# Saltfish-AB/LatentSync

Hardware: AMD Instinct MI355X
Metric: lip-synced frames/sec at 256x256, 16-frame window, 20 DDIM steps (higher is better)
Workload: dtype bf16; 1 GPU; configs[1]: 256x256 x16-frame windows, 20 DDIM steps, guidance 1.0, LatentSync-1.5 UNet + SD-VAE, bf16; 48 independent windows of a clip batched per UNet call; windows_per_rank=240, windows_per_batch=48, frames_per_window=16, global_batch=768, resolution=256, parallelism=dp1 (window sharding, RCCL all-gather of decoded frames)

## Files before the change

### latentsync_amd/build.py

```python
import concurrent.futures as cf
import os
import re
import shutil
import subprocess
import sys
import tempfile
import warnings

HERE = os.path.dirname(os.path.abspath(__file__))
REPO = os.path.dirname(HERE)
CSRC = os.path.join(HERE, "csrc")
OBJ = os.path.join(REPO, "build", "obj")
LIB = os.path.join(HERE, "libls_hip.so")
HIPCC = os.environ.get("HIPCC", "/opt/rocm/bin/hipcc")
FLAGS = ["--offload-arch=gfx950", "-O3", "-fPIC", "-std=c++17", "-Wno-unused-result", "-munsafe-fp-atomics",
         "-fno-slp-vectorize"]


def _deps():
    hdrs = [os.path.join(CSRC, f) for f in os.listdir(CSRC) if f.endswith(".h")]
    hdrs.append(os.path.join(REPO, "include", "ls_hip.h"))
    return max(os.path.getmtime(h) for h in hdrs)


COUNTED_VMCNT = ("gemm_rowblock_kernel", "conv_gemm_dma_kernel", "attn5_kernel", "attn8_kernel", "tattn_fused_kernel",
                 "attnw_kernel", "conv3x3_halo_kernel", "ff_chain_kernel")


def _spills(stderr):
    bad, cur = [], None
    for line in stderr.splitlines():
        m = re.search(r"remark: +Function Name: (\S+)", line)
        if m:
            cur = m.group(1)
            continue
        m = re.search(r"remark: +VGPRs Spill: (\d+)", line)
        if m and cur and int(m.group(1)) > 0 and any(k in cur for k in COUNTED_VMCNT):
            bad.append(f"{cur}: {line.split('remark:')[1].strip()}")
    return bad


OBJDUMP = os.environ.get("LLVM_OBJDUMP", "/opt/rocm/lib/llvm/bin/llvm-objdump")
_PK_OPSEL = re.compile(r"v_pk_\w+_f32\b[^\n]*\bop_sel:\[([01,]+)\]")


def _packed_opsel(obj):
    skip = os.environ.get("LS_SKIP_OPSEL_GUARD", "") not in ("", "0")
    if not os.path.exists(OBJDUMP):
        if skip:
            warnings.warn(f"packed-fp32 op_sel guard skipped (LS_SKIP_OPSEL_GUARD): {OBJDUMP} not found")
            return []
        raise RuntimeError(f"packed-fp32 op_sel guard: {OBJDUMP} not found (LS_SKIP_OPSEL_GUARD=1 to build without it)")
    with tempfile.TemporaryDirectory() as td:
        cp = os.path.join(td, "k.o")
        shutil.copy(obj, cp)
        r = subprocess.run([OBJDUMP, "--offloading", cp], capture_output=True, text=True, cwd=td)
        dev = [f for f in os.listdir(td) if "gfx950" in f]
        if r.returncode != 0 or not dev:
            msg = f"could not extract the gfx950 code object of {obj} ({r.stderr.strip()[:200]})"
            if skip:
                warnings.warn("packed-fp32 op_sel guard skipped (LS_SKIP_OPSEL_GUARD): " + msg)
                return []
            raise RuntimeError("packed-fp32 op_sel guard: " + msg + " (LS_SKIP_OPSEL_GUARD=1 to build without it)")
        r = subprocess.run([OBJDUMP, "-d", "--mcpu=gfx950", os.path.join(td, dev[0])], capture_output=True, text=True)
    return [m.group(0).split("//")[0].strip() for m in _PK_OPSEL.finditer(r.stdout) if "1" in m.group(1)]


def _compile(src, obj, dep_time):
    if os.path.exists(obj) and os.path.getmtime(obj) >= max(os.path.getmtime(src), dep_time):
        return obj, None
    cmd = [HIPCC] + FLAGS + ["-Rpass-analysis=kernel-resource-usage", "-c", src, "-o", obj]
    r = subprocess.run(cmd, capture_output=True, text=True)
    if r.returncode != 0:
        return obj, r.stderr
    with open(obj[:-2] + ".remarks", "w") as f:
        f.write(r.stderr)
    bad = _spills(r.stderr)
    if bad:
        os.remove(obj)
        return obj, "register spills in counted-vmcnt kernels:\n" + "\n".join(bad)
    try:
        bad = _packed_opsel(obj)
    except RuntimeError as e:
        os.remove(obj)
        return obj, str(e)
    if bad:
        os.remove(obj)
        return obj, f"{len(bad)} packed-fp32 op_sel instructions (wrong beside MFMAs on gfx950), e.g.:\n" + "\n".join(bad[:4])
    return obj, None


def build(verbose=True):
    os.makedirs(OBJ, exist_ok=True)
    srcs = sorted(os.path.join(CSRC, f) for f in os.listdir(CSRC) if f.endswith(".hip"))
    dep_time = _deps()
    objs = []
    with cf.ThreadPoolExecutor(max_workers=min(8, len(srcs))) as ex:
        futs = [ex.submit(_compile, s, os.path.join(OBJ, os.path.basename(s)[:-4] + ".o"), dep_time) for s in srcs]
        for f in futs:
            obj, err = f.result()
            if err:
                raise RuntimeError(f"hipcc failed for {obj}:\n{err}")
            objs.append(obj)
    if not os.path.exists(LIB) or os.path.getmtime(LIB) < max(os.path.getmtime(o) for o in objs):
        cmd = [HIPCC, "--offload-arch=gfx950", "-shared", "-fPIC", "-o", LIB] + objs
        r = subprocess.run(cmd, capture_output=True, text=True)
        if r.returncode != 0:
            raise RuntimeError("link failed:\n" + r.stderr)
        if verbose:
            print("built", LIB)
    return LIB


if __name__ == "__main__":
    build()
    sys.exit(0)
```

### latentsync_amd/csrc/ls_gemm.hip

```cpp
#include <type_traits>

#include "ls_common.h"

namespace ls {

struct ConvArgs {
  const u16* x1; const u16* x2;
  int C1, C2, Cin, ld1, ld2;
  int n_img, H, W, Ho, Wo, stride, pad, upsample;
  const float* aff_scale; const float* aff_shift; int pix_per_sample; int silu_in;
  const u16* w; int K, N, M, CC;
  const float* bias; const float* rowvec; int rows_per_vec, rowvec_ld, rowvec_mod;
  const float* ln_mr; const float* ln_cs;
  const u16* res; int ldr; float out_scale; int act;
  void* y; int ldy; int y_f32;
  int ktiles, kt_per_split, split; float* partial;
  int ntm, ntn;
  float* stats_out; float stats_eps;
  float* cs_out;
  int ablate;
  int ccm;
  int gm;
  int Mo;
  int phase;
// ... 1642 lines not shown
      if (b == 0 && ci > 0) load_par(ci);
    }
  };
  auto put_halo = [&](int buf, int j0, int j1, const uint4* v_in) __attribute__((always_inline)) {
    uint4* const hb0 = hbuf + buf * HALO;
    float4 gsc[2], gsh[2];
    if constexpr (GN) {
      const float4* gq = gpar + buf * 32 + hc8 * 2;
      gsc[0] = gq[0]; gsc[1] = gq[1]; gsh[0] = gq[16]; gsh[1] = gq[17];
    }
#pragma unroll
    for (int j = j0; j < j1; ++j) {
      if (j * NT + tid >= NPC) continue;
      uint4 v = v_in[j - j0];
      if constexpr (GN) {
        if (hpix[j] >= 0) {
          float f[8];
          unpack8(v, f);
          const float scl[8] = {gsc[0].x, gsc[0].y, gsc[0].z, gsc[0].w, gsc[1].x, gsc[1].y, gsc[1].z, gsc[1].w};
          const float shf[8] = {gsh[0].x, gsh[0].y, gsh[0].z, gsh[0].w, gsh[1].x, gsh[1].y, gsh[1].z, gsh[1].w};
#pragma unroll
          for (int e = 0; e < 8; ++e) f[e] = silu_log2(fmaf(f[e], scl[e], shf[e]));
          v = pack8(f);
        }
      }
      hb0[hdst[j]] = v;
    }
  };
  auto store_halo = [&](int buf, int b) { put_halo(buf, hb_lo(b, NHL), hb_lo(b + 1, NHL), hreg); };

  int wvo[DPT];
#pragma unroll
  for (int j = 0; j < DPT; ++j) {
    const int q = j * NT + tid, row = q >> 3, pc = q & 7;
    const int lc = pc ^ ((row >> 1) & 7);
    wvo[j] = ((q < WSLOT ? row : 0) * a.K + lc * 8) * 2;
  }
  auto wslot = [&](int par, int t) { return PH ? (NSW == 3 ? (par + t) % 3 : t & 1) : NSW == 3 ? t % 3 : (t & 1) ^ par; };
  const int wid_u = __builtin_amdgcn_readfirstlane(wid);
  __builtin_assume(wid_u >= 0 && wid_u < NT / 64);
  lds_u4* const wbuf_l = (lds_u4*)lds_dyn + 2 * HALO;
  lds_u4* const dummy_l = wbuf_l + NSW * WSLOT;
  auto issue_w = [&](int g, int sl) {
    lds_u4* slot = wbuf_l + sl * WSLOT + wid_u * 64;
#pragma unroll
    for (int j = 0; j < DPT; ++j) {
      const bool live = WSLOT % NT == 0 || j * NT + wid_u * 64 < WSLOT;
      ls_raw_buffer_load_lds(rs_w, (__attribute__((address_space(3))) void*)(live ? slot + j * NT : dummy_l), 16, wvo[j],
                             g * 128, 0, 0);
    }
  };

  static_assert(TW == 16, "fragment i = one patch row");
  const int p0 = 64 * wm + l16;
  const int hp0 = (p0 / TW) * P + (p0 % TW) + (COMPACT ? 0 : 3) + py * P + px;

  f32x4 acc[FM][FN];
#pragma unroll
  for (int i = 0; i < FM; ++i)
#pragma unroll
    for (int j = 0; j < FN; ++j) acc[i][j] = (f32x4){0.f, 0.f, 0.f, 0.f};

  for (int g = 0; g < NSW - 1 && g < G; ++g) issue_w(g, g % NSW);
  {
    uint4 hpre[NHL];
    if constexpr (GN) load_par(0);
#pragma unroll
    for (int j = 0; j < NHL; ++j) {
      const int vo = hpix[j] >= 0 ? hpix[j] * a.ld1 * 2 + hc8 * 16 : (int)0x80000000;
      hpre[j] = __builtin_bit_cast(uint4, ls_raw_buffer_load_v4(rs1, vo, 0, 0));
    }
    if constexpr (GN) {
      store_par(0);
      __syncthreads();
    }
    put_halo(0, 0, NHL, hpre);
  }

  bf16x8 apf[2][FM];
  auto read_a = [&](const uint4* hb, int tt) {
    constexpr int TPR = PH ? 2 : 3;
    const int hpt = hp0 + (tt / TPR) * P + tt % TPR;
    const int sw = COMPACT ? (l16 + px + tt % TPR) & 7 : hpt & 7;
#pragma unroll
    for (int ks = 0; ks < 2; ++ks) {
      const int base = hpt * 8 + ((ks * 4 + lg) ^ sw);
#pragma unroll
      for (int i = 0; i < FM; ++i)
        apf[ks][i] = __builtin_bit_cast(bf16x8, hb[base + 8 * (((16 * i) / TW) * P + (16 * i) % TW)]);
    }
  };
  auto tap = [&](int ci, int par, auto t_tag, auto last_tag) {
    constexpr int t = decltype(t_tag)::value;
    constexpr bool LAST = decltype(last_tag)::value;
    const int g = NTAP * ci + t;
    const int hpar = ci & 1;
    constexpr int HY = LAST ? 0 : (t - 1 >= 0 ? halo_issue(t - 1, NHL, GN, TS) : 0) +
                                  (NSW >= 3 && t - 2 >= 0 ? halo_issue(t - 2, NHL, GN, TS) : 0);
    if (g + NSW - 2 >= G) wait_vm<0>();
    else wait_vm<(NSW - 2) * DPT + HY>();
    asm volatile("s_waitcnt lgkmcnt(0)" ::: "memory");
    __builtin_amdgcn_s_barrier();
    asm volatile("" ::: "memory");
    if (g + NSW - 1 < G) issue_w(g + NSW - 1, wslot(par, t + NSW - 1));
    if constexpr (!LAST) {
      if constexpr (GN && t == 1) store_par(ci + 1);
      if constexpr (t == TS || t == 2 * TS) store_halo(hpar ^ 1, t / TS - 1);
      if constexpr (t == 0 || t == TS || t == 2 * TS) load_halo(ci + 1, t / TS);
    }
    const uint4* hb = hbuf + hpar * HALO;
    const uint4* wb = wbuf + wslot(par, t) * WSLOT;
    if constexpr (t == 0) read_a(hb, 0);
#pragma unroll
    for (int ks = 0; ks < 2; ++ks) {
      bf16x8 bfr[FN];
#pragma unroll
      for (int j = 0; j < FN; ++j)
        bfr[j] = __builtin_bit_cast(bf16x8, wb[swz64(wn * WTN + j * 16 + l16, ks * 4 + lg)]);
#pragma unroll
      for (int i = 0; i < FM; ++i)
#pragma unroll
        for (int j = 0; j < FN; ++j)
          acc[i][j] = __builtin_amdgcn_mfma_f32_16x16x32_bf16(apf[ks][i], bfr[j], acc[i][j], 0, 0, 0);
    }
    if constexpr (t < NTAP - 1) read_a(hb, t + 1);
    if constexpr (!LAST && t == NTAP - 1) store_halo(hpar ^ 1, 2);
  };
  using I0 = std::integral_constant<int, 0>; using I1 = std::integral_constant<int, 1>;
  using I2 = std::integral_constant<int, 2>; using I3 = std::integral_constant<int, 3>;
  using I4 = std::integral_constant<int, 4>; using I5 = std::integral_constant<int, 5>;
  using I6 = std::integral_constant<int, 6>; using I7 = std::integral_constant<int, 7>;
  using I8 = std::integral_constant<int, 8>;
  auto chunk = [&](int ci, auto last) {
    const int par = PH && NSW == 3 ? ci % 3 : ci & 1;
    tap(ci, par, I0{}, last); tap(ci, par, I1{}, last); tap(ci, par, I2{}, last);
    tap(ci, par, I3{}, last);
    if constexpr (!PH) {
      tap(ci, par, I4{}, last); tap(ci, par, I5{}, last);
      tap(ci, par, I6{}, last); tap(ci, par, I7{}, last); tap(ci, par, I8{}, last);
    }
  };
  for (int ci = 0; ci + 1 < nchunk; ++ci) chunk(ci, std::false_type{});
  chunk(nchunk - 1, std::true_type{});
  asm volatile("s_waitcnt lgkmcnt(0)" ::: "memory");
  __builtin_amdgcn_s_barrier();
  asm volatile("" ::: "memory");
  const int m0v = PH ? (int)(img * 4 * HW) + ((ph * tpc + tyb) * tpr + txb) * (TH * TW)
                     : (int)(img * HW) + (tyb * tpr + txb) * (TH * TW);
  const long m0r = PH ? img * 4 * HW + (long)(2 * y0 + py) * a.Wo + 2 * x0 + px : img * HW + (long)y0 * a.W + x0;
  static_assert((size_t)(NT / (BN / 8)) * BN * 2 * 4 <= (size_t)2 * HALO * 16, "column-sum partials fit the halo images");
  store_tile_plain<TH * TW, BN, TH / 4, WNW, false, CSF, PH ? -TW : TW, 2>(a, acc, (float*)lds_dyn, m0v, n0, m0r);
}

static bool g_force_regstage = false;
static int g_force_tile = 0, g_force_split = 0;
static int g_ablate = 0;

struct ConvPlan {
  ConvArgs a;
  ls_conv_plan_info i;
  float* cs_pass;
  float* row_stats;
};

template <int V>
using IC = std::integral_constant<int, V>;

template <void (*KERN)(ConvArgs)>
static void launch_plan(const ConvPlan& p, hipStream_t s) {
  if (p.i.lds_bytes) LS_SET_MAX_DYN_SHM(KERN, p.i.lds_bytes);
  KERN<<<p.i.grid, p.i.threads, p.i.lds_bytes, s>>>(p.a);
}

static bool vec_ok(const ConvArgs& a) { return a.N % 8 == 0 && a.ldy % 8 == 0 && (!a.res || a.ldr % 8 == 0); }

struct TileCfg { int bm, bn, split; };

static TileCfg pick_tile(long M, int N, int ktiles, bool allow_split, bool big_ok, int ksize) {
  struct Cand { int bm, bn; double eff; int waves, resident; };
  const Cand cands[] = {{128, 128, 1.0, 4, 2}, {128, 160, 1.2, 4, 2}, {128, 64, 0.72, 4, 2}, {64, 64, 0.42, 4, 4},
                        {128, 32, 0.36, 4, 4}, {256, 256, 1.5, 8, 1}};
  TileCfg best{128, 128, 1};
  double best_t = 1e300;
  for (const Cand& c : cands) {
    if (c.bn == 32 && N > 32) continue;
    if (N <= 32 && c.bn != 32) continue;
    if (c.bm == 256) {
      if (!big_ok || N < 256) continue;
      if (ksize == 1 && ((N % 256 != 0 && N < 1920) || (N < 1280 && N % 160 == 0))) continue;
    }
    if (c.bn == 160 && N % 160 != 0) continue;
    const long tiles = (long)cdiv(M, c.bm) * cdiv(N, c.bn);
    for (int split = 1; split <= 16; ++split) {
      if (split > 1 && (!allow_split || ktiles / split < 4 || tiles >= 256)) break;
      const long blocks = tiles * split;
      const long per_cu = (blocks + 255) / 256;
      const long conc = std::min<long>(c.resident, per_cu);
      const double f = (c.waves * conc >= 8) ? 1.0 : 0.75;
      const double per_block = (double)c.bm * c.bn * 64.0 * cdiv(ktiles, split) / c.eff;
      double t = per_cu * per_block / f;
      if (split > 1) t += (double)M * N * split * 1.5;
      if (t < best_t * 0.97) { best_t = t; best = {c.bm, c.bn, split}; }
    }
  }
  return best;
}

static void set_split(ConvArgs& a, int split) {
  a.kt_per_split = cdiv(a.ktiles, std::max(1, std::min(split, a.ktiles)));
  a.split = cdiv(a.ktiles, a.kt_per_split);
}

static bool g_rowblock = true;
static bool g_rowblock640 = true;
static bool g_rb640_res = false;
static bool g_rb640_fm2 = true;

static bool rowblock_ok(const ls_conv_desc* d, const ConvArgs& a) {
  if (!g_rowblock || g_force_tile || g_force_regstage || d->ksize != 1 || a.C2) return false;
  if (a.aff_scale && (a.ln_mr || a.silu_in || a.pix_per_sample % (a.Cin == 320 ? 256 : 128) ||
                      ((uintptr_t)a.aff_scale | (uintptr_t)a.aff_shift) & 15))
    return false;
  if (!((a.Cin == 320 && a.K == 320 && a.M % 256 == 0) ||
        (g_rowblock640 && a.Cin == 640 && a.K == 640 && a.M % 128 == 0 && (!a.res || g_rb640_res))))
    return false;
  if (a.N % 64 || a.split != 1 || a.y_f32) return false;
  if (a.act != LS_ACT_NONE && a.act != LS_ACT_GEGLU) return false;
  if (a.ldy % 4 || (a.res && a.ldr % 8) || (a.rowvec && (a.rowvec_ld % 4 || a.rows_per_vec % 256))) return false;
  if (((uintptr_t)a.y & 7) || ((uintptr_t)a.res & 15)) return false;
  return (((uintptr_t)a.x1 | (uintptr_t)a.bias | (uintptr_t)a.ln_cs | (uintptr_t)a.rowvec) & 15) == 0;
}

using RowblockInstances =
    std::integer_sequence<int, 0, RB_LN, RB_LN | RB_RV, RB_RES, RB_LN | RB_RES, RB_LN | RB_GEGLU, RB_GEGLU, RB_STATS,
                          RB_RES | RB_STATS, RB_RES | RB_GNCS, RB_AFF, RB_AFF | RB_STATS>;
constexpr int RB_FM1 = RB_STATS | RB_GNCS | RB_AFF;

constexpr size_t rowblock_lds(int kt, int fm, int flags) {
  return (size_t)3 * (16 * 2 * (kt / 2) * 8 + 48 + ((flags & RB_RES) ? 128 * fm * 16 * 2 / 8 : 0)) * 16 +
         ((flags & RB_GNCS) ? 4096 : 0);
}

template <int... F>
static bool rowblock_compiled(int flags, std::integer_sequence<int, F...>) {
  return ((flags == F) || ...);
}

static bool plan_rowblock(ConvPlan& p) {
  ConvArgs& a = p.a;
  const int flags = (a.ln_mr ? RB_LN : 0) | (a.res ? RB_RES : 0) | (a.rowvec ? RB_RV : 0) |
                    (a.act == LS_ACT_GEGLU ? RB_GEGLU : 0) | (a.stats_out ? RB_STATS : 0) | (a.cs_out ? RB_GNCS : 0) |
                    (a.aff_scale ? RB_AFF : 0);
  const int fm = a.K == 320 || (g_rb640_fm2 && !(flags & RB_FM1)) ? 2 : 1, bm = 128 * fm;
  if (a.M % bm || !rowblock_compiled(flags, RowblockInstances{})) return false;
  const int ntm = a.M / bm, nch = a.N / 32;
  const int ntn = std::max(1, std::min(nch, (256 + ntm - 1) / ntm));
  if ((a.stats_out || a.cs_out) && ntn != 1) return false;
  a.ntm = ntm;
  a.ntn = ntn;
  p.i.family = 1;
  p.i.rb_kt = a.K / 32;
  p.i.rb_fm = fm;
  p.i.rb_flags = flags;
  p.i.grid = ntm * ntn;
  p.i.threads = 512;
  p.i.lds_bytes = (int)rowblock_lds(p.i.rb_kt, fm, flags);
  return true;
}

template <int FLAGS>
static void launch_rowblock1(const ConvPlan& p, hipStream_t s) {
  if (p.i.rb_kt == 10) return launch_plan<gemm_rowblock_kernel<10, 2, 2, FLAGS>>(p, s);
  if constexpr (!(FLAGS & RB_FM1)) {
    if (p.i.rb_fm == 2) return launch_plan<gemm_rowblock_kernel<20, 2, 2, FLAGS>>(p, s);
  }
  launch_plan<gemm_rowblock_kernel<20, 1, 2, FLAGS>>(p, s);
}

template <int... F>
static void launch_rowblock(const ConvPlan& p, hipStream_t s, std::integer_sequence<int, F...>) {
  ((p.i.rb_flags == F ? launch_rowblock1<F>(p, s) : void()), ...);
}

constexpr size_t tiled_lds(int bm, int bn, int wm) {
  return std::max<size_t>((size_t)2 * (bm + bn) * 8 * 16, (size_t)(bm / wm) * (bn + 4) * 4);
}

static int epi_kind(const ConvArgs& a) {
  if (a.phase) return EPI_PLAINP;
  if (a.split != 1 || !vec_ok(a) || a.y_f32) return EPI_ANY;
  if (a.act == LS_ACT_NONE) return EPI_PLAIN;
  if (a.act == LS_ACT_GEGLU) return EPI_GEGLU;
  return EPI_ANY;
}

static bool buf_dma_ok(const ConvArgs& a, int ks) {
  if (a.aff_scale) return false;
  if (ks == 1) return a.Cin % 64 == 0 && a.C1 % 64 == 0 && a.K == a.Cin;
  if (a.upsample) return a.Cin % 64 == 0 && a.C1 % 64 == 0 && a.stride == 1 && a.pad == 1;
  return a.Cin % 64 == 0 && a.C1 % 64 == 0 && (a.stride == 1 || a.stride == 2) && (a.pad == 0 || a.pad == 1);
}

template <class B, class F>
static void with_epi(int epi, B buf, F f) {
  switch (epi) {
    case EPI_PLAIN: return f(IC<EPI_PLAIN>{}, buf);
    case EPI_GEGLU: return f(IC<EPI_GEGLU>{}, buf);
    default: return f(IC<EPI_ANY>{}, buf);
  }
}

template <int KS, bool TAPU, class F>
static void with_epi_buf(const ls_conv_plan_info& i, F f) {
  if constexpr (KS == 3 && TAPU) {
    if (i.epi == EPI_PLAINP) return f(IC<EPI_PLAINP>{}, std::true_type{});
  }
  if constexpr (KS == 1 || TAPU) {
    if (i.buf) return with_epi(i.epi, std::true_type{}, f);
  }
  with_epi(i.epi, std::false_type{}, f);
}

template <int BM, int BN, int WM, int WN, int KS, bool TAPU>
static void launch_tiled2(const ConvPlan& p, hipStream_t s) {
  if constexpr (BM != 256) {
    if (p.i.family == 2) return launch_plan<conv_gemm_kernel<BM, BN, WM, WN, KS, TAPU>>(p, s);
  }
  with_epi_buf<KS, TAPU>(p.i, [&](auto epi, auto buf) {
    constexpr int EPI = decltype(epi)::value;
    constexpr bool BUF = decltype(buf)::value;
    if constexpr (BM == 256) launch_plan<conv_gemm_big_kernel<BN, KS, TAPU, EPI, BUF>>(p, s);
    else launch_plan<conv_gemm_dma_kernel<BM, BN, WM, WN, KS, TAPU, EPI, BUF>>(p, s);
  });
}

template <int BM, int BN, int WM, int WN>
static void launch_tiled1(const ConvPlan& p, hipStream_t s) {
  if (p.i.ks == 1) launch_tiled2<BM, BN, WM, WN, 1, false>(p, s);
  else if (p.i.tapu) launch_tiled2<BM, BN, WM, WN, 3, true>(p, s);
  else launch_tiled2<BM, BN, WM, WN, 3, false>(p, s);
}

static void launch_tiled(const ConvPlan& p, hipStream_t s) {
  const int bm = p.i.bm, bn = p.i.bn;
  if (bm == 256 && bn == 256) launch_tiled1<256, 256, 2, 4>(p, s);
  else if (bm == 256) launch_tiled1<256, 128, 2, 4>(p, s);
  else if (bm == 128 && bn == 128) launch_tiled1<128, 128, 2, 2>(p, s);
  else if (bm == 128 && bn == 160) launch_tiled1<128, 160, 2, 2>(p, s);
  else if (bm == 128 && bn == 64) launch_tiled1<128, 64, 2, 2>(p, s);
  else if (bm == 128 && bn == 32) launch_tiled1<128, 32, 4, 1>(p, s);
  else launch_tiled1<64, 64, 2, 2>(p, s);
}

static bool tiled_phase_ok(const ConvArgs& a) {
  return a.upsample == 2 && vec_ok(a) && !a.y_f32 && a.act == LS_ACT_NONE && !a.rowvec && !a.C2 && !g_force_regstage &&
         buf_dma_ok(a, 3);
}

static void to_tiled_phase(ConvArgs& a, int bm) {
  a.phase = 1;
  a.upsample = 0;
  a.Ho = a.H;
  a.Wo = a.W;
  a.M = a.n_img * a.H * a.W;
  a.ntm = cdiv(a.M, bm);
  a.gm = std::max(1, std::min(a.gm, a.ntm));
}

static bool g_halo = true;
static bool g_halo_ups = true;
static bool g_halo_bn128 = false;
static bool g_halo_narrow = true;
static bool g_halo_th8 = true;

static bool halo_ok(const ls_conv_desc* d, const ConvArgs& a) {
  if (!g_halo || g_force_tile || g_force_regstage || d->ksize != 3 || a.stride != 1 || a.pad != 1 ||
      !a.ccm || a.Cin % 64 || a.C1 % 64 || a.K != (a.upsample == 2 ? 4 : 9) * a.Cin || a.y_f32 || a.act != LS_ACT_NONE ||
      a.ln_mr || a.stats_out || a.ldy % 8 || (a.res && a.ldr % 8))
    return false;
  if (a.upsample ? (!g_halo_ups || a.aff_scale || a.Ho != 2 * a.H || a.Wo != 2 * a.W) : (a.Ho != a.H || a.Wo != a.W))
    return false;
  const bool narrow = a.N % 8 == 0 && a.N <= 16 && a.H % 8 == 0 && g_halo_narrow;
  if (((a.N % 160 && a.N % 128) || a.N > 640) && !narrow) return false;
  if (a.aff_scale && (!a.silu_in || a.pix_per_sample % (a.H * a.W) || ((uintptr_t)a.aff_scale | (uintptr_t)a.aff_shift) & 15))
    return false;
  if (((uintptr_t)a.x1 | (uintptr_t)a.x2 | (uintptr_t)a.w) & 15 || a.ld1 % 8 || (a.C2 && a.ld2 % 8)) return false;
  if (a.upsample == 2 ? a.W % 16 || a.H % 16 : a.Wo % 16 || a.Ho % 16) return false;
  if (a.upsample == 2 && (a.N <= 16 || a.C2)) return false;
  if ((long)a.H * a.W * a.ld1 * 2 >= (1L << 31) || (a.C2 && (long)a.H * a.W * a.ld2 * 2 >= (1L << 31)))
    return false;
  return true;
}

template <class F>
static void with_halo_tile(const ls_conv_plan_info& i, F f) {
  if (i.halo_bn == 16) f(IC<16>{}, IC<8>{});
  else if (i.halo_bn == 160) f(IC<160>{}, IC<16>{});
  else if (i.halo_th == 8) f(IC<128>{}, IC<8>{});
  else f(IC<128>{}, IC<16>{});
}

static void plan_halo(ConvPlan& p) {
  ConvArgs& a = p.a;
  ls_conv_plan_info& i = p.i;
  i.halo_ph = a.upsample == 2;
  i.family = i.halo_ph ? 4 : 3;
  if (i.halo_ph) {
    a.upsample = 0;
  } else if (a.upsample) {
    a.H = a.Ho;
    a.W = a.Wo;
  }
  i.halo_bn = a.N <= 16 ? 16 : (a.N % 160 == 0 && !(g_halo_bn128 && a.N % 128 == 0)) ? 160 : 128;
  i.halo_th = i.halo_bn == 16 || (i.halo_bn == 128 && g_halo_th8 && a.Cin <= 256) ? 8 : 16;
  i.halo_gn = a.aff_scale != nullptr;
  i.halo_cs = a.cs_out != nullptr;
  with_halo_tile(i, [&](auto bn, auto th) {
    using HC = HaloCfg<16, decltype(bn)::value, decltype(th)::value>;
    i.threads = HC::NT;
    i.lds_bytes = (int)HC::SHM;
  });
  i.grid = a.n_img * (a.H / i.halo_th) * (a.W / 16) * cdiv(a.N, i.halo_bn) * (i.halo_ph ? 4 : 1);
}

template <int BN, int TH, bool PH>
static void launch_halo2(const ConvPlan& p, hipStream_t s) {
  if constexpr (!PH) {
    if (p.i.halo_gn)
      return p.i.halo_cs ? launch_plan<conv3x3_halo_kernel<16, BN, true, true, TH>>(p, s)
                         : launch_plan<conv3x3_halo_kernel<16, BN, true, false, TH>>(p, s);
  }
  p.i.halo_cs ? launch_plan<conv3x3_halo_kernel<16, BN, false, true, TH, PH>>(p, s)
              : launch_plan<conv3x3_halo_kernel<16, BN, false, false, TH, PH>>(p, s);
}

static void launch_halo(const ConvPlan& p, hipStream_t s) {
  with_halo_tile(p.i, [&](auto bn, auto th) {
    constexpr int BN = decltype(bn)::value, TH = decltype(th)::value;
    if constexpr (BN != 16) {
      if (p.i.halo_ph) return launch_halo2<BN, TH, true>(p, s);
    }
    launch_halo2<BN, TH, false>(p, s);
  });
}

static int plan_conv(const ls_conv_desc* d, ConvPlan& p) {
  if (!d || !d->x1 || !d->w || !d->y) return fail(LS_ERR_INVALID, "ls_conv2d: null pointer");
  if (d->ksize != 1 && d->ksize != 3) return fail(LS_ERR_INVALID, "ls_conv2d: ksize must be 1 or 3");
  const int Cin = d->C1 + d->C2;
  if (d->C1 % 8 || d->C2 % 8 || Cin <= 0) return fail(LS_ERR_INVALID, "ls_conv2d: channels must be multiples of 8");
  if (d->C2 && !d->x2) return fail(LS_ERR_INVALID, "ls_conv2d: C2 > 0 needs x2");
  if (d->ld1 % 8 || (d->C2 && d->ld2 % 8)) return fail(LS_ERR_INVALID, "ls_conv2d: pixel pitch must be a multiple of 8");
  if (d->upsample < 0 || d->upsample > 2) return fail(LS_ERR_INVALID, "ls_conv2d: upsample must be 0, 1 or 2");
  if (d->upsample == 2 && (d->ksize != 3 || Cin % 64 || d->K != 4 * Cin || d->aff_scale || d->stride != 1 ||
                           d->pad != 1 || d->Ho != 2 * d->H || d->Wo != 2 * d->W))
    return fail(LS_ERR_INVALID, "ls_conv2d: upsample 2 (phase-packed weights) needs ksize 3, Cin % 64 == 0, K == 4 Cin, "
                                "no affine prologue, stride 1, pad 1, Ho x Wo = 2H x 2W");
  const long Kneed = (d->upsample == 2 ? 4L : (long)d->ksize * d->ksize) * Cin;
  if (d->K % 64 || d->K < Kneed || d->K - Kneed >= 64)
    return fail(LS_ERR_INVALID, "ls_conv2d: K must be ksize^2*Cin rounded up to 64");
  if (d->ksize == 1 && (d->Ho != d->H || d->Wo != d->W || d->stride != 1 || d->upsample))
    return fail(LS_ERR_INVALID, "ls_conv2d: ksize 1 must be stride 1 with no resampling");
  if (d->act == LS_ACT_GEGLU && (d->N % 32)) return fail(LS_ERR_INVALID, "ls_conv2d: GEGLU needs N % 32 == 0");
  if (d->act == LS_ACT_GEGLU && (d->rowvec || d->res || (d->out_scale != 0.f && d->out_scale != 1.f)))
    return fail(LS_ERR_INVALID, "ls_conv2d: GEGLU takes no rowvec, residual or out_scale");
  if (d->aff_scale && (!d->aff_shift || d->imgs_per_sample <= 0))
    return fail(LS_ERR_INVALID, "ls_conv2d: affine prologue needs shift and imgs_per_sample");
  if (d->rowvec && d->rows_per_vec <= 0) return fail(LS_ERR_INVALID, "ls_conv2d: rowvec needs rows_per_vec");
  const long M = (long)d->n_img * d->Ho * d->Wo;
  if (M <= 0 || M >= (1L << 31)) return fail(LS_ERR_INVALID, "ls_conv2d: bad M");
  p = ConvPlan{};
  ConvArgs& a = p.a;
  a.x1 = d->x1; a.x2 = d->x2; a.C1 = d->C1; a.C2 = d->C2; a.Cin = Cin; a.ld1 = d->ld1; a.ld2 = d->ld2;
  a.n_img = d->n_img; a.H = d->H; a.W = d->W; a.Ho = d->Ho; a.Wo = d->Wo;
  a.stride = d->stride; a.pad = d->pad; a.upsample = d->upsample;
  a.aff_scale = d->aff_scale; a.aff_shift = d->aff_shift;
  a.pix_per_sample = d->imgs_per_sample * d->H * d->W; a.silu_in = d->silu_in;
  a.w = d->w; a.K = d->K; a.N = d->N; a.M = (int)M; a.Mo = (int)M; a.phase = 0; a.CC = Cin / 8;
  a.bias = d->bias; a.rowvec = d->rowvec; a.rows_per_vec = d->rows_per_vec; a.rowvec_mod = d->rowvec_mod;
  a.ln_mr = d->ln_rowstats; a.ln_cs = d->ln_colsum;
  if (a.ln_mr && (!a.ln_cs || d->ksize != 1)) return fail(LS_ERR_INVALID, "ls_conv2d: ln_rowstats needs ln_colsum, ksize 1");
  a.rowvec_ld = d->rowvec_ld > 0 ? d->rowvec_ld : d->N;
  a.res = d->res; a.ldr = d->ldr; a.out_scale = d->out_scale == 0.f ? 1.f : d->out_scale; a.act = d->act;
  a.y = d->y; a.ldy = d->ldy; a.y_f32 = d->y_f32;
  a.stats_out = d->row_stats_out;
  a.stats_eps = d->row_stats_eps > 0.f ? d->row_stats_eps : 1e-5f;
  if (a.stats_out && (d->ksize != 1 || d->act == LS_ACT_GEGLU || d->y_f32))
    return fail(LS_ERR_INVALID, "ls_conv2d: row_stats_out needs ksize 1, bf16 output, no GEGLU");
  a.cs_out = d->gn_colsum_out;
  if (a.cs_out && (M % CS_ROWS || d->N % 8 || d->ldy % 8 || d->act == LS_ACT_GEGLU || d->y_f32))
    return fail(LS_ERR_INVALID, "ls_conv2d: gn_colsum_out needs M % 128 == 0, N % 8 == 0, bf16 output, no GEGLU");
  a.ablate = g_ablate;
  a.ccm = (d->ksize == 3 && Cin % 64 == 0) ? 1 : 0;
  a.ktiles = d->K / 64;
  TileCfg t = pick_tile(M, d->N, a.ktiles, d->split_k <= 0 && d->workspace != nullptr && d->upsample != 2,
                        !d->aff_scale && !g_force_regstage && (d->ksize == 1 || Cin % 64 == 0), d->ksize);
  if (g_force_tile) {
    static const int tb[10][2] = {{0, 0}, {128, 128}, {128, 64}, {64, 64}, {128, 32}, {256, 256}, {256, 128},
                                  {0, 0}, {0, 0}, {128, 160}};
    t.bm = tb[g_force_tile][0]; t.bn = tb[g_force_tile][1]; t.split = g_force_split ? g_force_split : 1;
    if (t.bm >= 256 && (d->aff_scale || g_force_regstage)) { t.bm = 128; t.bn = 128; }
  }
  a.ntm = cdiv(M, t.bm); a.ntn = cdiv(d->N, t.bn);
  a.gm = 1;
  if (t.bm == 256 && t.bn == 256 && d->ksize == 1 && d->K <= 1920) a.gm = 4;
  a.gm = std::max(1, std::min(a.gm, a.ntm));
  set_split(a, d->upsample == 2 ? 1 : d->split_k > 0 ? d->split_k : t.split);
  const size_t slab = (size_t)a.M * a.N * sizeof(float);
  ls_conv_plan_info& i = p.i;
  i.bm = i.bn = i.ks = i.tapu = i.buf = i.epi = i.rb_kt = i.rb_fm = i.rb_flags = -1;
  i.halo_bn = i.halo_th = i.halo_gn = i.halo_cs = i.halo_ph = -1;
  i.workspace_bytes = a.split > 1 ? (int64_t)(a.split * slab) : 0;
  if (a.split > 1 && (!d->workspace || d->workspace_bytes < a.split * slab))
    set_split(a, d->workspace ? (int)std::min<size_t>(d->workspace_bytes / slab, a.split) : 1);
  if (a.split > 1) a.partial = (float*)d->workspace;

  float* const cs = a.cs_out;
  float* const stats = a.stats_out;
  bool planned = false;
  if (halo_ok(d, a)) {
    plan_halo(p);
    planned = true;
  } else if (a.upsample == 2) {
    if (!tiled_phase_ok(a))
      return fail(LS_ERR_INVALID, "ls_conv2d: no phase-form kernel for this shape (ls_conv_path -1): use upsample = 1");
    to_tiled_phase(a, t.bm);
  } else if (rowblock_ok(d, a)) {
    for (int round = 0; round < 4 && !planned; ++round) {
      const bool fuse_stats = round < 2, fuse_cs = round % 2 == 0;
      if ((!fuse_stats && !stats) || (!fuse_cs && !cs)) continue;
      a.stats_out = fuse_stats ? stats : nullptr;
      a.cs_out = fuse_cs ? cs : nullptr;
      planned = plan_rowblock(p);
    }
    if (planned) {
      p.cs_pass = a.cs_out ? nullptr : cs;
      p.row_stats = a.stats_out ? nullptr : stats;
    }
  }
  if (!planned) {
    const bool regstage = a.aff_scale || g_force_regstage;
    const bool cs_epi = cs && !a.phase && a.split == 1 && vec_ok(a) && !(t.bm == 128 && t.bn == 32) && t.bm != 64 && t.bm < 256;
    a.cs_out = cs_epi ? cs : nullptr;
    a.stats_out = nullptr;
    p.cs_pass = cs_epi ? nullptr : cs;
    p.row_stats = stats;
    i.family = a.phase ? 5 : regstage ? 2 : 0;
    i.bm = t.bm;
    i.bn = t.bn;
    i.ks = d->ksize;
    i.tapu = d->ksize == 3 && Cin % 64 == 0;
    i.buf = !regstage && buf_dma_ok(a, d->ksize);
    i.epi = regstage ? -1 : epi_kind(a);
    i.grid = a.ntm * a.ntn * (a.phase ? 4 : a.split);
    i.threads = t.bm == 256 ? 512 : 256;
    i.lds_bytes = regstage ? 0 : (int)tiled_lds(t.bm, t.bn, t.bn == 32 ? 4 : 2);
    i.reduce = a.split > 1;
  }
  i.split = a.split;
  i.colsum_rows = p.cs_pass ? a.Mo : 0;
  i.row_stats = p.row_stats != nullptr;
  return LS_OK;
}

}

using namespace ls;

extern "C" int ls_set_tuning(int32_t key, int32_t value) {
  switch (key) {
    case 18: g_halo_ups = value != 0; return LS_OK;
    case 19: g_halo_narrow = value != 0; return LS_OK;
    case 20: g_rb640_res = value != 0; return LS_OK;
    case 17:
      if (value != 1) return fail(LS_ERR_INVALID, "ls_ff_chain rows per wave: 1 (16) only");
      return LS_OK;
    case 1: g_force_regstage = value != 0; return LS_OK;
    case 2:
      if (value < 0 || value > 9 || value == 7 || value == 8) return fail(LS_ERR_INVALID, "tile id 0..6 or 9");
      g_force_tile = value;
      return LS_OK;
    case 3: g_force_split = value; return LS_OK;
    case 4: g_ablate = value; return LS_OK;
    case 6: g_rowblock = value != 0; return LS_OK;
    case 7: g_rowblock640 = value != 0; return LS_OK;
    case 8: g_halo = value != 0; return LS_OK;
    case 12:
      if (!value) return fail(LS_ERR_INVALID, "key 12 = 0 (padded halo rows) no longer exists");
      return LS_OK;
    case 13: g_halo_bn128 = value != 0; return LS_OK;
    case 15: g_rb640_fm2 = value != 0; return LS_OK;
    case 16: g_halo_th8 = value != 0; return LS_OK;
    case 9:
      if (value) return fail(LS_ERR_INVALID, "attention variant: 0 only");
      return LS_OK;
    default: return fail(LS_ERR_INVALID, "ls_set_tuning: unknown key");
  }
}

template <typename K>
static int occ(K kern, int threads, size_t shm) {
  int n = 0;
  (void)hipFuncSetAttribute((const void*)kern, hipFuncAttributeMaxDynamicSharedMemorySize, (int)shm);
  if (hipOccupancyMaxActiveBlocksPerMultiprocessor(&n, kern, threads, shm) != hipSuccess) return -1;
  return n;
}

extern "C" int ls_gemm_occupancy(int32_t which) {
  switch (which) {
    case 1: return occ(conv_gemm_dma_kernel<128, 160, 2, 2, 1, false, EPI_PLAIN>, 256, tiled_lds(128, 160, 2));
    case 2: return occ(conv_gemm_big_kernel<256, 1, false, EPI_PLAIN>, 512, tiled_lds(256, 256, 2));
    case 3: return occ(conv_gemm_dma_kernel<128, 128, 2, 2, 1, false, EPI_PLAIN>, 256, tiled_lds(128, 128, 2));
    default: return fail(LS_ERR_INVALID, "ls_gemm_occupancy: which 1..3");
  }
}

extern "C" int ls_conv_plan(const ls_conv_desc* d, ls_conv_plan_info* out) {
  ConvPlan p;
  if (!out) return fail(LS_ERR_INVALID, "ls_conv_plan: null out");
  const int rc = plan_conv(d, p);
  if (rc == LS_OK) *out = p.i;
  return rc;
}

extern "C" int ls_conv_path(const ls_conv_desc* d) {
  ConvPlan p;
  return plan_conv(d, p) == LS_OK ? p.i.family : -1;
}

extern "C" size_t ls_conv_workspace_bytes(const ls_conv_desc* d) {
  ConvPlan p;
  return plan_conv(d, p) == LS_OK ? (size_t)p.i.workspace_bytes : 0;
}

extern "C" int ls_conv2d(const ls_conv_desc* d, void* stream) {
  ConvPlan p;
  int rc = plan_conv(d, p);
  if (rc != LS_OK) return rc;
  hipStream_t s = (hipStream_t)stream;
  const ConvArgs& a = p.a;
  const int f = p.i.family;
  if (f == 1) launch_rowblock(p, s, RowblockInstances{});
  else if (f == 3 || f == 4) launch_halo(p, s);
  else launch_tiled(p, s);
  rc = check_launch(f == 1 ? "gemm_rowblock_kernel" : f == 3 || f == 4 ? "conv3x3_halo_kernel" : "conv_gemm_kernel");
  if (rc != LS_OK) return rc;
  if (p.i.reduce) {
    const long nchunk = (long)a.M * ((((a.act == LS_ACT_GEGLU) ? a.N / 2 : a.N) + 7) / 8);
    splitk_reduce_kernel<<<cdiv(nchunk, 256), 256, 0, s>>>(a);
    if ((rc = check_launch("splitk_reduce_kernel")) != LS_OK) return rc;
  }
  if (p.cs_pass && (rc = launch_colsum_pass((const u16*)a.y, a.ldy, p.i.colsum_rows, a.N, p.cs_pass, s)) != LS_OK) return rc;
  if (p.row_stats) return ls_row_stats((const uint16_t*)a.y, a.ldy, a.Mo, a.N, a.stats_eps, p.row_stats, stream);
  return LS_OK;
}

extern "C" int ls_gn_colsum(const uint16_t* y, int64_t ldy, int64_t M, int32_t N, float* out, void* stream) {
  return launch_colsum_pass(y, ldy, M, N, out, (hipStream_t)stream);
}
```

Measured before the change: 152.6 frames/s.

## Add persistent 3x3 halo conv kernel that prefetches next tile during last chunk

Adds a persistent variant of the 3x3 halo convolution kernel. It launches one block per CU, loops over output tiles, and overlaps the next tile's weight and halo loads with the last channel chunk of the current tile. The goal is to remove per-block launch and pipeline fill/drain costs on large-Cin convs without input affine, where there are at least four tiles per CU. In exchange it forces TH=16 tiles with one block per CU, which lowers occupancy, and it adds a complex cross-tile pipeline that risks synchronisation bugs.

```diff
diff --git a/latentsync_amd/build.py b/latentsync_amd/build.py
--- a/latentsync_amd/build.py
+++ b/latentsync_amd/build.py
@@ -24,7 +24,7 @@
 
 
 COUNTED_VMCNT = ("gemm_rowblock_kernel", "conv_gemm_dma_kernel", "attn5_kernel", "attn8_kernel", "tattn_fused_kernel",
-                 "attnw_kernel", "conv3x3_halo_kernel", "ff_chain_kernel")
+                 "attnw_kernel", "conv3x3_halo_kernel", "conv3x3_halo_persist_kernel", "ff_chain_kernel")
 
 
 def _spills(stderr):
diff --git a/latentsync_amd/csrc/ls_gemm.hip b/latentsync_amd/csrc/ls_gemm.hip
--- a/latentsync_amd/csrc/ls_gemm.hip
+++ b/latentsync_amd/csrc/ls_gemm.hip
@@ -1818,6 +1818,282 @@
   store_tile_plain<TH * TW, BN, TH / 4, WNW, false, CSF, PH ? -TW : TW, 2>(a, acc, (float*)lds_dyn, m0v, n0, m0r);
 }
 
+template <int BN, bool GN, bool CSF, bool PH = false>
+__global__ void __launch_bounds__((HaloCfg<16, BN, 16>::NT), 1) conv3x3_halo_persist_kernel(ConvArgs a) {
+  using HC = HaloCfg<16, BN, 16>;
+  static_assert(!(PH && GN), "the phase form takes no input affine");
+  static_assert(HC::NSW == 3 && !HC::COMPACT && HC::WSLOT % HC::NT == 0 && HC::WNW == 2, "the padded 3-slot form");
+  constexpr int TW = 16, TH = 16;
+  constexpr int NTAP = PH ? 4 : 9;
+  constexpr int P = HC::P, HALO = HC::HALO, WSLOT = HC::WSLOT, NT = HC::NT, NW = NT / 64;
+  constexpr int NRUN = HALO / 64;
+  constexpr int NHD = (NRUN + NW - 1) / NW;
+  constexpr int DPT = HC::DPT, FM = 4, FN = HC::FN, WNW = HC::WNW, WTN = BN / WNW;
+  static_assert(HALO % 64 == 0 && NW == 8, "whole runs, run r = 8 j + wave");
+  static_assert(PH || NHD > NTAP - 4, "a run per tap from tap 3, the rest at the last tap");
+  static_assert((size_t)64 * (BN + 4) * 4 <= (size_t)HALO * 16, "epilogue staging fits ONE halo image");
+  static_assert((size_t)(NT / (BN / 8)) * BN * 2 * 4 <= (size_t)HALO * 16, "column-sum partials fit one halo image");
+  extern __shared__ __attribute__((aligned(16))) uint4 lds_dyn[];
+  uint4* const hbuf = lds_dyn;
+  uint4* const wbuf = lds_dyn + 2 * HALO;
+  uint4* const dummy = wbuf + 3 * WSLOT;
+  float4* const gpar = (float4*)(dummy + 64);
+
+  const int tid = threadIdx.x, lane = tid & 63, wid = tid >> 6;
+  int wn, l16, lg, hp0;
+  const int ntn = (a.N + BN - 1) / BN, tpr = a.W / TW, tpc = a.H / TH;
+  const int T = a.n_img * tpc * tpr * ntn * (PH ? 4 : 1);
+  const int Gb = gridDim.x;
+  int L = blockIdx.x;
+  if (L >= T) return;
+  const long HW = (long)a.H * a.W;
+  const int ups = a.upsample;
+  const int Wi = a.W >> ups;
+  const long HWi = HW >> (2 * ups);
+  const int nchunk = a.Cin / 64;
+  const int G = NTAP * nchunk;
+  const uint32_t cap = 0x7FFFFFFFu;
+  const int wid_u = __builtin_amdgcn_readfirstlane(wid);
+  __builtin_assume(wid_u >= 0 && wid_u < NW);
+
+  struct Tile { int tn, ph, txb, tyb, img; };
+  auto decode = [&](int l) {
+    int b = xcd_remap(l, T);
+    Tile t;
+    t.tn = b % ntn;
+    b /= ntn;
+    t.ph = 0;
+    if constexpr (PH) {
+      t.ph = b & 3;
+      b >>= 2;
+    }
+    t.txb = b % tpr;
+    b /= tpr;
+    t.tyb = b % tpc;
+    t.img = b / tpc;
+    return t;
+  };
+  auto wdesc = [&](const Tile& t) {
+    const int n0 = t.tn * BN;
+    return buffer_rsrc(a.w + ((long)t.ph * a.N + n0) * a.K, (uint32_t)min((long)min(BN, a.N - n0) * a.K * 2, (long)cap));
+  };
+
+  const int lc = (lane & 7) ^ (lane >> 3);
+  int hoff[NHD];
+  i32x4 rs1p, rs2p;
+  long affp;
+  auto aim = [&](const Tile& t) {
+    const int y0 = t.tyb * TH, x0 = t.txb * TW;
+    int tid_a = tid;
+    asm volatile("" : "+v"(tid_a));
+#pragma unroll
+    for (int j = 0; j < NHD; ++j) {
+      const int r = j * NW + wid_u, slot = j * NT / 8 + (tid_a >> 3);
+      const int hr = slot / P, hcol = slot - hr * P - 3;
+      const int y = y0 - 1 + hr, x = x0 - 1 + hcol;
+      hoff[j] = r < NRUN && hcol >= 0 && hcol < TW + 2 && y >= 0 && y < a.H && x >= 0 && x < a.W
+                    ? (y >> ups) * Wi + (x >> ups) : -1;
+    }
+    rs1p = buffer_rsrc(a.x1 + t.img * HWi * a.ld1, (uint32_t)min((long)HWi * a.ld1 * 2, (long)cap));
+    rs2p = a.C2 ? buffer_rsrc(a.x2 + t.img * HWi * a.ld2, (uint32_t)min((long)HWi * a.ld2 * 2, (long)cap)) : rs1p;
+    affp = (long)t.img * HW / a.pix_per_sample * a.Cin;
+  };
+  lds_u4* const hbuf_l = (lds_u4*)lds_dyn;
+  lds_u4* const wbuf_l = hbuf_l + 2 * HALO;
+  lds_u4* const dummy_l = wbuf_l + 3 * WSLOT;
+  auto issue_h = [&](int ci, int j0, int j1, int buf) {
+    const bool two = ci * 64 >= a.C1;
+    const int ld = two ? a.ld2 : a.ld1;
+    const int soff = (two ? ci * 64 - a.C1 : ci * 64) * 2;
+    lds_u4* const run = hbuf_l + buf * HALO + wid_u * 64;
+#pragma unroll
+    for (int j = j0; j < j1; ++j) {
+      const bool live = j * NW + wid_u < NRUN;
+      const int vo = hoff[j] >= 0 ? hoff[j] * ld * 2 + lc * 16 : (int)0x80000000;
+      ls_raw_buffer_load_lds(two ? rs2p : rs1p, (__attribute__((address_space(3))) void*)(live ? run + j * NT : dummy_l), 16,
+                             vo, soff, 0, 0);
+    }
+  };
+  float4 gp;
+  auto load_par = [&](int ci) {
+    const int k = tid & 31;
+    gp = *(const float4*)((k < 16 ? a.aff_scale : a.aff_shift) + affp + ci * 64 + (k & 15) * 4);
+  };
+  auto store_par = [&](int buf) {
+    constexpr float L2E = 1.4426950408889634f;
+    if (tid < 32) gpar[buf * 32 + tid] = make_float4(gp.x * L2E, gp.y * L2E, gp.z * L2E, gp.w * L2E);
+  };
+  auto transform = [&](int buf, int j0, int j1) __attribute__((always_inline)) {
+    uint4* const hb0 = hbuf + buf * HALO + wid_u * 64 + lane;
+    const float4* gq = gpar + buf * 32 + lc * 2;
+    const float4 gsc0 = gq[0], gsc1 = gq[1], gsh0 = gq[16], gsh1 = gq[17];
+    const float scl[8] = {gsc0.x, gsc0.y, gsc0.z, gsc0.w, gsc1.x, gsc1.y, gsc1.z, gsc1.w};
+    const float shf[8] = {gsh0.x, gsh0.y, gsh0.z, gsh0.w, gsh1.x, gsh1.y, gsh1.z, gsh1.w};
+#pragma unroll
+    for (int j = j0; j < j1; ++j) {
+      if (hoff[j] < 0) continue;
+      float f[8];
+      unpack8(hb0[j * NT], f);
+#pragma unroll
+      for (int e = 0; e < 8; ++e) f[e] = silu_log2(fmaf(f[e], scl[e], shf[e]));
+      hb0[j * NT] = pack8(f);
+    }
+  };
+
+  int wvo[DPT];
+#pragma unroll
+  for (int j = 0; j < DPT; ++j) {
+    const int q = j * NT + tid, row = q >> 3, pc = q & 7;
+    const int lcw = pc ^ ((row >> 1) & 7);
+    wvo[j] = (row * a.K + lcw * 8) * 2;
+  }
+  auto wslot = [&](int par, int t) { return PH ? (par + t) % 3 : t % 3; };
+  auto issue_w = [&](const i32x4& rs, int g, int sl) {
+    lds_u4* slot = wbuf_l + sl * WSLOT + wid_u * 64;
+#pragma unroll
+    for (int j = 0; j < DPT; ++j)
+      ls_raw_buffer_load_lds(rs, (__attribute__((address_space(3))) void*)(slot + j * NT), 16, wvo[j], g * 128, 0, 0);
+  };
+
+  f32x4 acc[FM][FN];
+#pragma unroll
+  for (int i = 0; i < FM; ++i)
+#pragma unroll
+    for (int j = 0; j < FN; ++j) acc[i][j] = (f32x4){0.f, 0.f, 0.f, 0.f};
+
+  Tile cur = decode(L), nxt = cur;
+  i32x4 rs_w = wdesc(cur), rs_wn = rs_w;
+  aim(cur);
+  issue_w(rs_w, 0, wslot(0, 0));
+  issue_w(rs_w, 1, wslot(0, 1));
+  if constexpr (GN) load_par(0);
+  issue_h(0, 0, NHD, 0);
+  if constexpr (GN) store_par(0);
+  wait_vm<0>();
+  if constexpr (GN) {
+    __syncthreads();
+    transform(0, 0, NHD);
+  }
+
+  bf16x8 apf[2][FM];
+  auto read_a = [&](const uint4* hb, int tt) {
+    constexpr int TPR = PH ? 2 : 3;
+    const int hpt = hp0 + (tt / TPR) * P + tt % TPR;
+    const int sw = hpt & 7;
+#pragma unroll
+    for (int ks = 0; ks < 2; ++ks) {
+      const int base = hpt * 8 + ((ks * 4 + lg) ^ sw);
+#pragma unroll
+      for (int i = 0; i < FM; ++i) apf[ks][i] = __builtin_bit_cast(bf16x8, hb[base + 8 * i * P]);
+    }
+  };
+  auto tap = [&](int ci, int nci, int hpar, int par, bool fresh, auto t_tag, auto last_tag) {
+    constexpr int t = decltype(t_tag)::value;
+    constexpr bool LAST = decltype(last_tag)::value;
+    const int g = NTAP * ci + t;
+    constexpr int HY = LAST ? 0 : (t == 1 || t == 2 ? NHD + (GN ? 1 : 0) : 0);
+    if ((LAST && g + 1 >= G) || (t == 0 && fresh)) wait_vm<0>();
+    else wait_vm<DPT + HY>();
+    asm volatile("s_waitcnt lgkmcnt(0)" ::: "memory");
+    __builtin_amdgcn_s_barrier();
+    asm volatile("" ::: "memory");
+    if (g + 2 < G) issue_w(rs_w, g + 2, wslot(par, t + 2));
+    else if constexpr (!LAST) issue_w(rs_wn, g + 2 - G, wslot(par, t + 2));
+    auto side = [&]() __attribute__((always_inline)) {
+      if constexpr (!LAST) {
+        if constexpr (t == 0) {
+          if constexpr (GN) load_par(nci);
+          issue_h(nci, 0, NHD, hpar ^ 1);
+        }
+        if constexpr (GN && t == 1) store_par(hpar ^ 1);
+        if constexpr (GN && t >= 3 && t < NTAP - 1) transform(hpar ^ 1, t - 3, t - 2);
+        if constexpr (GN && t == NTAP - 1) transform(hpar ^ 1, NTAP - 4, NHD);
+      }
+    };
+    if (wid_u < NW / 2) side();
+    const uint4* hb = hbuf + hpar * HALO;
+    const uint4* wb = wbuf + wslot(par, t) * WSLOT;
+    if constexpr (t == 0) read_a(hb, 0);
+#pragma unroll
+    for (int ks = 0; ks < 2; ++ks) {
+      bf16x8 bfr[FN];
+#pragma unroll
+      for (int j = 0; j < FN; ++j)
+        bfr[j] = __builtin_bit_cast(bf16x8, wb[swz64(wn * WTN + j * 16 + l16, ks * 4 + lg)]);
+#pragma unroll
+      for (int i = 0; i < FM; ++i)
+#pragma unroll
+        for (int j = 0; j < FN; ++j)
+          acc[i][j] = __builtin_amdgcn_mfma_f32_16x16x32_bf16(apf[ks][i], bfr[j], acc[i][j], 0, 0, 0);
+    }
+    if constexpr (t < NTAP - 1) read_a(hb, t + 1);
+    if (wid_u >= NW / 2) side();
+  };
+  using I0 = std::integral_constant<int, 0>; using I1 = std::integral_constant<int, 1>;
+  using I2 = std::integral_constant<int, 2>; using I3 = std::integral_constant<int, 3>;
+  using I4 = std::integral_constant<int, 4>; using I5 = std::integral_constant<int, 5>;
+  using I6 = std::integral_constant<int, 6>; using I7 = std::integral_constant<int, 7>;
+  using I8 = std::integral_constant<int, 8>;
+  auto chunk = [&](int ci, int nci, int hpar, int par, bool fresh, auto last) {
+    tap(ci, nci, hpar, par, fresh, I0{}, last); tap(ci, nci, hpar, par, fresh, I1{}, last);
+    tap(ci, nci, hpar, par, fresh, I2{}, last); tap(ci, nci, hpar, par, fresh, I3{}, last);
+    if constexpr (!PH) {
+      tap(ci, nci, hpar, par, fresh, I4{}, last); tap(ci, nci, hpar, par, fresh, I5{}, last);
+      tap(ci, nci, hpar, par, fresh, I6{}, last); tap(ci, nci, hpar, par, fresh, I7{}, last);
+      tap(ci, nci, hpar, par, fresh, I8{}, last);
+    }
+  };
+  int hpar = 0, par3 = 0;
+  bool fresh = false;
+  for (;;) {
+    const bool more = L + Gb < T;
+    int tid_o = tid;
+    asm volatile("" : "+v"(tid_o));
+    {
+      const int lane_o = tid_o & 63, wid_o = tid_o >> 6;
+      wn = wid_o % WNW;
+      l16 = lane_o & 15;
+      lg = lane_o >> 4;
+      const int p0 = 64 * (wid_o / WNW) + l16;
+      hp0 = (p0 / TW) * P + (p0 % TW) + 3 + (cur.ph >> 1) * P + (cur.ph & 1);
+    }
+#pragma unroll 1
+    for (int ci = 0; ci < nchunk; ++ci) {
+      const bool lastc = ci + 1 == nchunk;
+      if (lastc && more) {
+        nxt = decode(L + Gb);
+        rs_wn = wdesc(nxt);
+        aim(nxt);
+      }
+      if (lastc && !more) chunk(ci, 0, hpar, par3, fresh, std::true_type{});
+      else chunk(ci, lastc ? 0 : ci + 1, hpar, par3, fresh, std::false_type{});
+      fresh = false;
+      hpar ^= 1;
+      par3 = par3 == 2 ? 0 : par3 + 1;
+    }
+    asm volatile("s_waitcnt lgkmcnt(0)" ::: "memory");
+    __builtin_amdgcn_s_barrier();
+    asm volatile("" ::: "memory");
+    const int y0 = cur.tyb * TH, x0 = cur.txb * TW, py = cur.ph >> 1, px = cur.ph & 1;
+    const int m0v = PH ? (int)(cur.img * 4 * HW) + ((cur.ph * tpc + cur.tyb) * tpr + cur.txb) * (TH * TW)
+                       : (int)(cur.img * HW) + (cur.tyb * tpr + cur.txb) * (TH * TW);
+    const long m0r = PH ? cur.img * 4 * HW + (long)(2 * y0 + py) * a.Wo + 2 * x0 + px : cur.img * HW + (long)y0 * a.W + x0;
+    int tid_e = tid;
+    asm volatile("" : "+v"(tid_e));
+    store_tile_plain<TH * TW, BN, TH / 4, WNW, false, CSF, PH ? -TW : TW, 2>(a, acc, (float*)(hbuf + (hpar ^ 1) * HALO), m0v,
+                                                                           cur.tn * BN, m0r, tid_e);
+    if (!more) break;
+    L += Gb;
+    cur = nxt;
+    rs_w = rs_wn;
+    fresh = true;
+#pragma unroll
+    for (int i = 0; i < FM; ++i)
+#pragma unroll
+      for (int j = 0; j < FN; ++j) acc[i][j] = (f32x4){0.f, 0.f, 0.f, 0.f};
+  }
+}
+
 static bool g_force_regstage = false;
 static int g_force_tile = 0, g_force_split = 0;
 static int g_ablate = 0;
@@ -1827,6 +2103,7 @@
   ls_conv_plan_info i;
   float* cs_pass;
   float* row_stats;
+  bool halo_persist;
 };
 
 template <int V>
@@ -2038,6 +2315,20 @@
 static bool g_halo_bn128 = false;
 static bool g_halo_narrow = true;
 static bool g_halo_th8 = true;
+static int g_halo_persist = 1, g_halo_persist_cap = 0;
+
+static int device_cus() {
+  static const int n = [] {
+    int dev = 0, cu = 0;
+    if (hipGetDevice(&dev) != hipSuccess ||
+        hipDeviceGetAttribute(&cu, hipDeviceAttributeMultiprocessorCount, dev) != hipSuccess) {
+      (void)hipGetLastError();
+      return 0;
+    }
+    return cu;
+  }();
+  return n;
+}
 
 static bool halo_ok(const ls_conv_desc* d, const ConvArgs& a) {
   if (!g_halo || g_force_tile || g_force_regstage || d->ksize != 3 || a.stride != 1 || a.pad != 1 ||
@@ -2058,6 +2349,10 @@
   return true;
 }
 
+static bool halo_persist_pick(const ConvArgs& a, int tiles, int grid) {
+  return !a.aff_scale && a.Cin >= 512 && tiles >= 4 * grid;
+}
+
 template <class F>
 static void with_halo_tile(const ls_conv_plan_info& i, F f) {
   if (i.halo_bn == 16) f(IC<16>{}, IC<8>{});
@@ -2081,12 +2376,28 @@
   i.halo_th = i.halo_bn == 16 || (i.halo_bn == 128 && g_halo_th8 && a.Cin <= 256) ? 8 : 16;
   i.halo_gn = a.aff_scale != nullptr;
   i.halo_cs = a.cs_out != nullptr;
+  const int tiles16 = a.n_img * (a.H / 16) * (a.W / 16) * cdiv(a.N, 128) * (i.halo_ph ? 4 : 1);
+  const int pgrid = g_halo_persist_cap > 0 ? g_halo_persist_cap : device_cus();
+  p.halo_persist = i.halo_bn == 128 && pgrid > 0 && (g_halo_persist == 2 || (g_halo_persist == 1 && halo_persist_pick(a, tiles16, pgrid)));
+  if (p.halo_persist) i.halo_th = 16;
   with_halo_tile(i, [&](auto bn, auto th) {
     using HC = HaloCfg<16, decltype(bn)::value, decltype(th)::value>;
     i.threads = HC::NT;
     i.lds_bytes = (int)HC::SHM;
   });
   i.grid = a.n_img * (a.H / i.halo_th) * (a.W / 16) * cdiv(a.N, i.halo_bn) * (i.halo_ph ? 4 : 1);
+  if (p.halo_persist) i.grid = std::min(tiles16, pgrid);
+}
+
+template <bool PH>
+static void launch_halo_persist(const ConvPlan& p, hipStream_t s) {
+  if constexpr (!PH) {
+    if (p.i.halo_gn)
+      return p.i.halo_cs ? launch_plan<conv3x3_halo_persist_kernel<128, true, true>>(p, s)
+                         : launch_plan<conv3x3_halo_persist_kernel<128, true, false>>(p, s);
+  }
+  p.i.halo_cs ? launch_plan<conv3x3_halo_persist_kernel<128, false, true, PH>>(p, s)
+              : launch_plan<conv3x3_halo_persist_kernel<128, false, false, PH>>(p, s);
 }
 
 template <int BN, int TH, bool PH>
@@ -2101,6 +2412,7 @@
 }
 
 static void launch_halo(const ConvPlan& p, hipStream_t s) {
+  if (p.halo_persist) return p.i.halo_ph ? launch_halo_persist<true>(p, s) : launch_halo_persist<false>(p, s);
   with_halo_tile(p.i, [&](auto bn, auto th) {
     constexpr int BN = decltype(bn)::value, TH = decltype(th)::value;
     if constexpr (BN != 16) {
@@ -2257,6 +2569,14 @@
     case 13: g_halo_bn128 = value != 0; return LS_OK;
     case 15: g_rb640_fm2 = value != 0; return LS_OK;
     case 16: g_halo_th8 = value != 0; return LS_OK;
+    case 22:
+      if (value < 0 || value > 2) return fail(LS_ERR_INVALID, "persistent halo conv: 0 off, 1 per shape, 2 wherever it applies");
+      g_halo_persist = value;
+      return LS_OK;
+    case 23:
+      if (value < 0) return fail(LS_ERR_INVALID, "persistent halo conv grid: blocks >= 0 (0: one per CU)");
+      g_halo_persist_cap = value;
+      return LS_OK;
     case 9:
       if (value) return fail(LS_ERR_INVALID, "attention variant: 0 only");
       return LS_OK;
```

Result: no change. 152.8 frames/s (median of 6 runs) (+0.1%).
